# NUS-HPC-AI-Lab/VideoSys

Measured on AMD Instinct MI355X. Metric: videos/min (Open-Sora 512x512x64f, 30 denoise steps, DiT denoising only) + sec/denoise-step, higher is better.
Workload: dtype bf16; 1 GPU; open-sora-v1.2 STDiT3-XL/2 512x512x64f, latent [4,19,64,64], CFG batch 2 = 38912 token rows, 300 text tokens, depth 28; steps_per_video=30, parallelism=dsp1

## Files before the change

### videosys_amd/csrc/rowwise.hip

```cpp
#include "common.h"

#include <cstdlib>
#include "vsys_internal.h"

namespace vsys {
namespace {

template <int MAXV>
__global__ __launch_bounds__(256) void adaln_modulate_kernel(const bf16_t* __restrict__ x, const bf16_t* __restrict__ shift,
                                                             const bf16_t* __restrict__ scale, bf16_t* __restrict__ y,
                                                             int64_t rows, int C, int64_t rows_per_sample,
                                                             int64_t mod_stride, float eps) {
  const int lane = threadIdx.x & 63;
  const int64_t row = (int64_t)blockIdx.x * 4 + (threadIdx.x >> 6);
  if (row >= rows) return;
  const int nchunk = C >> 3;
  const bf16_t* xr = x + row * C;
  float v[MAXV][8];
  float s = 0.f;
#pragma unroll
  for (int i = 0; i < MAXV; ++i) {
    const int c = lane + 64 * i;
    if (c < nchunk) {
      uint4 u = *reinterpret_cast<const uint4*>(xr + c * 8);
      unpack8(u, v[i]);
#pragma unroll
      for (int e = 0; e < 8; ++e) s += v[i][e];
    }
  }
  const float mean = wave_sum(s) / (float)C;
  float q = 0.f;
#pragma unroll
  for (int i = 0; i < MAXV; ++i) {
    const int c = lane + 64 * i;
    if (c < nchunk) {
#pragma unroll
      for (int e = 0; e < 8; ++e) {
        float d = v[i][e] - mean;
        q += d * d;
      }
    }
  }
  const float rstd = rsqrtf(wave_sum(q) / (float)C + eps);
  const int64_t b = row / rows_per_sample;
  const bf16_t* sh = shift + b * mod_stride;
  const bf16_t* sc = scale + b * mod_stride;
  bf16_t* yr = y + row * C;
#pragma unroll
  for (int i = 0; i < MAXV; ++i) {
    const int c = lane + 64 * i;
    if (c < nchunk) {
      float a[8], m[8], o[8];
      unpack8(*reinterpret_cast<const uint4*>(sh + c * 8), a);
      unpack8(*reinterpret_cast<const uint4*>(sc + c * 8), m);
#pragma unroll
      for (int e = 0; e < 8; ++e) o[e] = (v[i][e] - mean) * rstd * (1.0f + m[e]) + a[e];
      *reinterpret_cast<uint4*>(yr + c * 8) = pack8(o);
    }
  }
}

template <int RPW>
__global__ __launch_bounds__(256) void adaln_modulate_rows_kernel(const bf16_t* __restrict__ x, const bf16_t* __restrict__ shift,
                                                                  const bf16_t* __restrict__ scale, bf16_t* __restrict__ y,
                                                                  int64_t rows, int C, int64_t rows_per_sample,
                                                                  int64_t mod_stride, float eps) {
  constexpr int MAXV = 3;
  const int lane = threadIdx.x & 63;
  const int64_t row0 = ((int64_t)blockIdx.x * 4 + (threadIdx.x >> 6)) * RPW;
  if (row0 >= rows) return;
  const int nchunk = C >> 3;
  uint4 u[RPW][MAXV];
#pragma unroll
  for (int r = 0; r < RPW; ++r) {
    const int64_t row = row0 + r < rows ? row0 + r : rows - 1;
#pragma unroll
    for (int i = 0; i < MAXV; ++i) {
      const int c = lane + 64 * i;
      u[r][i] = c < nchunk ? *reinterpret_cast<const uint4*>(x + row * C + c * 8) : make_uint4(0, 0, 0, 0);
    }
  }
  const int64_t b = row0 / rows_per_sample;
  uint4 ush[MAXV], usc[MAXV];
#pragma unroll
  for (int i = 0; i < MAXV; ++i) {
    const int c = lane + 64 * i;
    ush[i] = c < nchunk ? *reinterpret_cast<const uint4*>(shift + b * mod_stride + c * 8) : make_uint4(0, 0, 0, 0);
    usc[i] = c < nchunk ? *reinterpret_cast<const uint4*>(scale + b * mod_stride + c * 8) : make_uint4(0, 0, 0, 0);
  }
#pragma unroll
  for (int r = 0; r < RPW; ++r) {
    float v[MAXV][8];
    float s = 0.f;
#pragma unroll
    for (int i = 0; i < MAXV; ++i) {
      unpack8(u[r][i], v[i]);
      if (lane + 64 * i < nchunk) {
#pragma unroll
        for (int e = 0; e < 8; ++e) s += v[i][e];
      }
    }
    const float mean = wave_sum(s) / (float)C;
    float q = 0.f;
#pragma unroll
    for (int i = 0; i < MAXV; ++i) {
      if (lane + 64 * i < nchunk) {
#pragma unroll
        for (int e = 0; e < 8; ++e) {
          float d = v[i][e] - mean;
          q += d * d;
        }
      }
    }
    const float rstd = rsqrtf(wave_sum(q) / (float)C + eps);
    if (row0 + r < rows) {
#pragma unroll
      for (int i = 0; i < MAXV; ++i) {
        const int c = lane + 64 * i;
        if (c < nchunk) {
          float a[8], m[8], o[8];
          unpack8(ush[i], a);
          unpack8(usc[i], m);
#pragma unroll
          for (int e = 0; e < 8; ++e) o[e] = (v[i][e] - mean) * rstd * (1.0f + m[e]) + a[e];
          *reinterpret_cast<uint4*>(y + (row0 + r) * C + c * 8) = pack8(o);
        }
      }
    }
  }
}

template <int MAXV>
__global__ __launch_bounds__(256) void ln_modulate_kernel(const bf16_t* __restrict__ x, const bf16_t* __restrict__ ln_w,
                                                          const bf16_t* __restrict__ ln_b, const bf16_t* __restrict__ shift,
                                                          const bf16_t* __restrict__ scale, bf16_t* __restrict__ y, int64_t rows,
                                                          int C, int64_t rows_per_sample, int64_t mod_stride, int64_t seg_split,
                                                          int64_t mod_alt, float eps) {
  const int lane = threadIdx.x & 63;
  const int64_t row = (int64_t)blockIdx.x * 4 + (threadIdx.x >> 6);
  if (row >= rows) return;
  const int nchunk = C >> 3;
  const bf16_t* xr = x + row * C;
  float v[MAXV][8];
  float s = 0.f;
#pragma unroll
  for (int i = 0; i < MAXV; ++i) {
    const int c = lane + 64 * i;
    if (c < nchunk) {
      unpack8(*reinterpret_cast<const uint4*>(xr + c * 8), v[i]);
#pragma unroll
      for (int e = 0; e < 8; ++e) s += v[i][e];
    }
  }
  const float mean = wave_sum(s) / (float)C;
  float q = 0.f;
#pragma unroll
  for (int i = 0; i < MAXV; ++i) {
    const int c = lane + 64 * i;
    if (c < nchunk) {
#pragma unroll
      for (int e = 0; e < 8; ++e) {
        const float d = v[i][e] - mean;
        q += d * d;
      }
    }
  }
  const float rstd = rsqrtf(wave_sum(q) / (float)C + eps);
  const int64_t b = row / rows_per_sample;
  const int64_t alt = (seg_split > 0 && row - b * rows_per_sample < seg_split) ? mod_alt : 0;
  bf16_t* yr = y + row * C;
#pragma unroll
  for (int i = 0; i < MAXV; ++i) {
    const int c = lane + 64 * i;
    if (c < nchunk) {
      float o[8];
#pragma unroll
      for (int e = 0; e < 8; ++e) o[e] = (v[i][e] - mean) * rstd;
      if (ln_w != nullptr) {
        float w[8], bb[8];
        unpack8(*reinterpret_cast<const uint4*>(ln_w + c * 8), w);
        unpack8(*reinterpret_cast<const uint4*>(ln_b + c * 8), bb);
#pragma unroll
        for (int e = 0; e < 8; ++e) o[e] = o[e] * w[e] + bb[e];
      }
      if (shift != nullptr) {
        float a[8], m[8];
        unpack8(*reinterpret_cast<const uint4*>(shift + b * mod_stride + alt + c * 8), a);
        unpack8(*reinterpret_cast<const uint4*>(scale + b * mod_stride + alt + c * 8), m);
#pragma unroll
        for (int e = 0; e < 8; ++e) o[e] = o[e] * (1.0f + m[e]) + a[e];
      }
      *reinterpret_cast<uint4*>(yr + c * 8) = pack8(o);
    }
  }
}

__global__ void gate_add_rows_kernel(bf16_t* __restrict__ x, const bf16_t* __restrict__ y, const bf16_t* __restrict__ gate,
                                     int64_t rows, int C8, int64_t rows_per_sample, int64_t gate_stride, int64_t seg_split,
                                     int64_t gate_alt) {
  const int64_t total = rows * C8;
  for (int64_t i = (int64_t)blockIdx.x * blockDim.x + threadIdx.x; i < total; i += (int64_t)gridDim.x * blockDim.x) {
    const int64_t r = i / C8;
    const int c = (int)(i - r * C8);
    const int64_t b = r / rows_per_sample;
    const int64_t alt = (seg_split > 0 && r - b * rows_per_sample < seg_split) ? gate_alt : 0;
    float a[8], v[8], g[8];
    unpack8(reinterpret_cast<const uint4*>(x)[i], a);
    unpack8(reinterpret_cast<const uint4*>(y)[i], v);
    unpack8(*reinterpret_cast<const uint4*>(gate + b * gate_stride + alt + c * 8), g);
#pragma unroll
    for (int k = 0; k < 8; ++k) a[k] += bf2f(f2bf(g[k] * v[k]));
    reinterpret_cast<uint4*>(x)[i] = pack8(a);
  }
}

__global__ void im2col_patch_kernel(const float* __restrict__ z, int Bz, bf16_t* __restrict__ out, int B, int F, int Cin, int H,
                                    int W, int p) {
  const int Hp = H / p, Wp = W / p, K = Cin * p * p;
  const int64_t total = (int64_t)B * F * Hp * Wp * K;
  for (int64_t i = (int64_t)blockIdx.x * blockDim.x + threadIdx.x; i < total; i += (int64_t)gridDim.x * blockDim.x) {
    const int k = (int)(i % K);
    const int64_t tok = i / K;
    const int wp = (int)(tok % Wp), hp = (int)((tok / Wp) % Hp), f = (int)((tok / ((int64_t)Wp * Hp)) % F);
    const int b = (int)(tok / ((int64_t)Wp * Hp * F));
    const int dx = k % p, dy = (k / p) % p, c = k / (p * p);
    out[i] = f2bf(z[((((int64_t)(b % Bz) * F + f) * Cin + c) * H + hp * p + dy) * W + wp * p + dx]);
  }
}

__global__ void unpatchify_cvx_kernel(const bf16_t* __restrict__ x, int64_t ldx, float* __restrict__ out, int B, int F, int Hp,
                                      int Wp, int Cout, int p) {
  const int H = Hp * p, W = Wp * p;
  const int64_t total = (int64_t)B * F * Cout * H * W;
  for (int64_t i = (int64_t)blockIdx.x * blockDim.x + threadIdx.x; i < total; i += (int64_t)gridDim.x * blockDim.x) {
    const int w = (int)(i % W), h = (int)((i / W) % H), c = (int)((i / ((int64_t)W * H)) % Cout);
    const int64_t bf = i / ((int64_t)W * H * Cout);
    const int64_t tok = (bf * Hp + h / p) * Wp + w / p;
    out[i] = bf2f(x[tok * ldx + (c * p + h % p) * p + w % p]);
  }
}

__global__ void mod_table_kernel(const bf16_t* __restrict__ table, const bf16_t* __restrict__ t_mlp, bf16_t* __restrict__ out,
                                 int nblk, int B, int C6) {
  const int64_t i = (int64_t)blockIdx.x * blockDim.x + threadIdx.x;
  const int64_t total = (int64_t)nblk * B * C6;
  if (i >= total) return;
  const int c = (int)(i % C6);
  const int b = (int)((i / C6) % B);
  const int k = (int)(i / ((int64_t)C6 * B));
  out[i] = f2bf(bf2f(table[(int64_t)k * C6 + c]) + bf2f(t_mlp[(int64_t)b * C6 + c]));
}

__global__ void timestep_embedding_kernel(const float* __restrict__ t, bf16_t* __restrict__ out, int B, int dim) {
  const int i = blockIdx.x * blockDim.x + threadIdx.x;
  const int half = dim / 2;
  if (i >= B * half) return;
  const int b = i / half, k = i - b * half;
  const float f = expf(-9.210340371976184f * (float)k / (float)half);
  const float a = t[b] * f;
  out[(int64_t)b * dim + k] = f2bf(cosf(a));
  out[(int64_t)b * dim + half + k] = f2bf(sinf(a));
}

__global__ __launch_bounds__(256) void patch_embed_kernel(const float* __restrict__ x, int Bz, const bf16_t* __restrict__ w,
                                                          const bf16_t* __restrict__ bias, const bf16_t* __restrict__ pos,
                                                          bf16_t* __restrict__ out, int B, int Cin, int T, int H, int W,
                                                          int ph, int pw, int C, int s0, int Sl) {
  const int Hp = (H + ph - 1) / ph, Wp = (W + pw - 1) / pw;
  const int S = Hp * Wp;
  const int cchunks = C >> 3;
  const int64_t total = (int64_t)B * T * Sl * cchunks;
  const int64_t i = (int64_t)blockIdx.x * blockDim.x + threadIdx.x;
  if (i >= total) return;
  const int cc = (int)(i % cchunks);
  const int64_t tok = i / cchunks;
  const int s = s0 + (int)(tok % Sl);
  const int t = (int)((tok / Sl) % T);
  const int b = (int)(tok / ((int64_t)Sl * T));
  const int bz = b % Bz;
  if (s >= S) {
    *reinterpret_cast<uint4*>(out + tok * C + cc * 8) = make_uint4(0, 0, 0, 0);
    return;
  }
  const int hp = s / Wp, wp = s - hp * Wp;
  float acc[8];
  {
    float bb[8];
    unpack8(*reinterpret_cast<const uint4*>(bias + cc * 8), bb);
#pragma unroll
    for (int e = 0; e < 8; ++e) acc[e] = bb[e];
  }
  const int K = Cin * ph * pw;
  if (K == 16) {
    float xin[16];
#pragma unroll
    for (int k = 0; k < 16; ++k) {
      const int ci = k >> 2, dy = (k >> 1) & 1, dx = k & 1;
      const int hh = hp * 2 + dy, ww = wp * 2 + dx;
      xin[k] = 0.f;
      if (ph == 2 && pw == 2 && hh < H && ww < W) xin[k] = bf2f(f2bf(x[((((int64_t)bz * Cin + ci) * T + t) * H + hh) * W + ww]));
    }
    if (ph == 2 && pw == 2) {
#pragma unroll
      for (int e = 0; e < 8; ++e) {
        const bf16_t* wr = w + (int64_t)(cc * 8 + e) * 16;
        float wa[8], wb[8];
        unpack8(*reinterpret_cast<const uint4*>(wr), wa);
        unpack8(*reinterpret_cast<const uint4*>(wr + 8), wb);
#pragma unroll
        for (int k = 0; k < 8; ++k) acc[e] += xin[k] * wa[k] + xin[k + 8] * wb[k];
      }
    }
  }
  if (!(K == 16 && ph == 2 && pw == 2)) {
    for (int ci = 0; ci < Cin; ++ci)
      for (int dy = 0; dy < ph; ++dy)
        for (int dx = 0; dx < pw; ++dx) {
          const int hh = hp * ph + dy, ww = wp * pw + dx;
          float xv = 0.f;
          if (hh < H && ww < W) xv = bf2f(f2bf(x[((((int64_t)bz * Cin + ci) * T + t) * H + hh) * W + ww]));
          const int k = (ci * ph + dy) * pw + dx;
#pragma unroll
          for (int e = 0; e < 8; ++e) acc[e] += xv * bf2f(w[(int64_t)(cc * 8 + e) * K + k]);
        }
  }
  float pp[8];
  unpack8(*reinterpret_cast<const uint4*>(pos + (int64_t)s * C + cc * 8), pp);
#pragma unroll
  for (int e = 0; e < 8; ++e) acc[e] = bf2f(f2bf(acc[e])) + pp[e];
  *reinterpret_cast<uint4*>(out + tok * C + cc * 8) = pack8(acc);
}

template <int MAXV>
__global__ __launch_bounds__(256) void final_layer_kernel(const bf16_t* __restrict__ x, const bf16_t* __restrict__ table,
                                                          const bf16_t* __restrict__ tvec, const bf16_t* __restrict__ w,
                                                          const bf16_t* __restrict__ bias, float* __restrict__ out,
                                                          int B, int T, int Hp, int Wp, int H, int W, int ph, int pw,
                                                          int Cout, int C, float eps, int Sl, float* __restrict__ tokens) {
  const int lane = threadIdx.x & 63;
  const int S = Sl;
  const int64_t rows = (int64_t)B * T * S;
  const int64_t row = (int64_t)blockIdx.x * 4 + (threadIdx.x >> 6);
  if (row >= rows) return;
  const int nchunk = C >> 3;
  const bf16_t* xr = x + row * C;
  float v[MAXV][8];
  float s = 0.f;
#pragma unroll
  for (int i = 0; i < MAXV; ++i) {
    const int c = lane + 64 * i;
    if (c < nchunk) {
      unpack8(*reinterpret_cast<const uint4*>(xr + c * 8), v[i]);
#pragma unroll
      for (int e = 0; e < 8; ++e) s += v[i][e];
    } else {
#pragma unroll
      for (int e = 0; e < 8; ++e) v[i][e] = 0.f;
    }
  }
  const float mean = wave_sum(s) / (float)C;
  float q = 0.f;
#pragma unroll
  for (int i = 0; i < MAXV; ++i) {
    const int c = lane + 64 * i;
    if (c < nchunk) {
#pragma unroll
      for (int e = 0; e < 8; ++e) {
        float d = v[i][e] - mean;
        q += d * d;
      }
    }
  }
  const float rstd = rsqrtf(wave_sum(q) / (float)C + eps);
  const int b = (int)(row / ((int64_t)T * S));
#pragma unroll
  for (int i = 0; i < MAXV; ++i) {
    const int c = lane + 64 * i;
    if (c < nchunk) {
      float sh[8], sc[8], tt[8];
      unpack8(*reinterpret_cast<const uint4*>(table + c * 8), sh);
      unpack8(*reinterpret_cast<const uint4*>(table + C + c * 8), sc);
      unpack8(*reinterpret_cast<const uint4*>(tvec + (int64_t)b * C + c * 8), tt);
#pragma unroll
      for (int e = 0; e < 8; ++e) {
        const float shift = bf2f(f2bf(sh[e] + tt[e])), scale = bf2f(f2bf(sc[e] + tt[e]));
        v[i][e] = bf2f(f2bf((v[i][e] - mean) * rstd * (1.0f + scale) + shift));
      }
    }
  }
  const int NOUT = ph * pw * Cout;
  const int64_t tok = row % ((int64_t)T * S);
  const int t = (int)(tok / S), sidx = (int)(tok % S);
  const int hp = sidx / Wp, wp = sidx - hp * Wp;
  for (int n = 0; n < NOUT; ++n) {
    const bf16_t* wr = w + (int64_t)n * C;
    float d = 0.f;
#pragma unroll
    for (int i = 0; i < MAXV; ++i) {
      const int c = lane + 64 * i;
      if (c < nchunk) {
        float ww[8];
        unpack8(*reinterpret_cast<const uint4*>(wr + c * 8), ww);
#pragma unroll
        for (int e = 0; e < 8; ++e) d += v[i][e] * ww[e];
      }
    }
    d = wave_sum(d);
    if (lane == 0) {
      d = bf2f(f2bf(d + bf2f(bias[n])));
      if (tokens != nullptr) {
        tokens[row * NOUT + n] = d;
        continue;
      }
      const int co = n % Cout;
      const int dx = (n / Cout) % pw, dy = n / (Cout * pw);
      const int hh = hp * ph + dy, ww2 = wp * pw + dx;
      if (hh < H && ww2 < W) out[((((int64_t)b * Cout + co) * T + t) * H + hh) * W + ww2] = d;
    }
  }
}

__global__ void unpatchify_tokens_kernel(const float* __restrict__ tok, float* __restrict__ out, int P, int B, int T, int Sl,
                                         int Hp, int Wp, int H, int W, int ph, int pw, int Cout) {
  const int NOUT = ph * pw * Cout;
  const int64_t total = (int64_t)B * Cout * T * H * W;
  const int64_t i = (int64_t)blockIdx.x * blockDim.x + threadIdx.x;
  if (i >= total) return;
  const int ww = (int)(i % W), hh = (int)((i / W) % H), t = (int)((i / ((int64_t)W * H)) % T);
  const int co = (int)((i / ((int64_t)W * H * T)) % Cout), b = (int)(i / ((int64_t)W * H * T * Cout));
  const int hp = hh / ph, dy = hh - hp * ph, wp = ww / pw, dx = ww - wp * pw;
  const int s = hp * Wp + wp;
  const int r = s / Sl, j = s - r * Sl;
  const int n = (dy * pw + dx) * Cout + co;
  out[i] = tok[((((int64_t)r * B + b) * T + t) * Sl + j) * NOUT + n];
}

__global__ void cfg_euler_kernel(float* __restrict__ z, const float* __restrict__ model_out, int Bz, int Cin, int Cout,
                                 int64_t thw, float guidance, float dt) {
  const int64_t i = (int64_t)blockIdx.x * blockDim.x + threadIdx.x;
  const int64_t total = (int64_t)Bz * Cin * thw;
  if (i >= total) return;
  const int64_t sp = i % thw;
  const int c = (int)((i / thw) % Cin);
  const int b = (int)(i / (thw * Cin));
  const float cond = model_out[((int64_t)b * Cout + c) * thw + sp];
  const float unc = model_out[((int64_t)(b + Bz) * Cout + c) * thw + sp];
  z[i] = z[i] + (unc + guidance * (cond - unc)) * dt;
}

__global__ void cfg_axpby_kernel(float* __restrict__ z, const float* __restrict__ model_out, int Bz, int Cin, int Cout,
                                 int64_t thw, float guidance, float c_z, float c_eps, int cond_first) {
  const int64_t i = (int64_t)blockIdx.x * blockDim.x + threadIdx.x;
  const int64_t total = (int64_t)Bz * Cin * thw;
  if (i >= total) return;
  const int64_t sp = i % thw;
  const int c = (int)((i / thw) % Cin);
  const int b = (int)(i / (thw * Cin));
  const float h0 = model_out[((int64_t)b * Cout + c) * thw + sp];
  const float h1 = model_out[((int64_t)(b + Bz) * Cout + c) * thw + sp];
  const float cond = cond_first ? h0 : h1, unc = cond_first ? h1 : h0;
  z[i] = c_z * z[i] + c_eps * (unc + guidance * (cond - unc));
}

__global__ void add_bcast_rows_kernel(bf16_t* __restrict__ x, const bf16_t* __restrict__ e, int64_t rows, int C8, int64_t group,
                                      int64_t period) {
  const int64_t total = rows * C8;
  for (int64_t i = (int64_t)blockIdx.x * blockDim.x + threadIdx.x; i < total; i += (int64_t)gridDim.x * blockDim.x) {
    const int64_t r = i / C8;
    const int c = (int)(i - r * C8);
    const int64_t er = (r / group) % period;
    float a[8], b[8];
    unpack8(reinterpret_cast<const uint4*>(x)[i], a);
    unpack8(reinterpret_cast<const uint4*>(e)[er * C8 + c], b);
#pragma unroll
    for (int k = 0; k < 8; ++k) a[k] += b[k];
    reinterpret_cast<uint4*>(x)[i] = pack8(a);
  }
}

__global__ void add_rows_kernel(bf16_t* __restrict__ x, const bf16_t* __restrict__ y, int64_t n8) {
  for (int64_t i = (int64_t)blockIdx.x * blockDim.x + threadIdx.x; i < n8; i += (int64_t)gridDim.x * blockDim.x) {
    float a[8], b[8];
    unpack8(reinterpret_cast<const uint4*>(x)[i], a);
    unpack8(reinterpret_cast<const uint4*>(y)[i], b);
#pragma unroll
    for (int e = 0; e < 8; ++e) a[e] += b[e];
    reinterpret_cast<uint4*>(x)[i] = pack8(a);
  }
}

__global__ void scale_add_rows_kernel(const bf16_t* __restrict__ a, int64_t lda, const bf16_t* __restrict__ b, int64_t ldb,
                                      bf16_t* __restrict__ out, int64_t ldo, int64_t rows, int C8, float scale) {
  const int64_t total = rows * C8;
  for (int64_t i = (int64_t)blockIdx.x * blockDim.x + threadIdx.x; i < total; i += (int64_t)gridDim.x * blockDim.x) {
    const int64_t r = i / C8;
    const int c = (int)(i - r * C8) * 8;
    float x[8], y[8];
    unpack8(*reinterpret_cast<const uint4*>(a + r * lda + c), x);
    unpack8(*reinterpret_cast<const uint4*>(b + r * ldb + c), y);
#pragma unroll
    for (int e = 0; e < 8; ++e) x[e] = bf2f(f2bf(x[e] * scale)) + y[e];
    *reinterpret_cast<uint4*>(out + r * ldo + c) = pack8(x);
  }
}

__global__ void copy_4d_kernel(const bf16_t* __restrict__ src, bf16_t* __restrict__ dst, int n0, int n1, int n2, int C,
                               int64_t ss0, int64_t ss1, int64_t ss2, int64_t ds0, int64_t ds1, int64_t ds2,
                               int n1_valid, int n2_valid) {
  const int cch = C >> 3;
  const int64_t total = (int64_t)n0 * n1 * n2 * cch;
  for (int64_t i = (int64_t)blockIdx.x * blockDim.x + threadIdx.x; i < total; i += (int64_t)gridDim.x * blockDim.x) {
    const int c = (int)(i % cch);
    int64_t r = i / cch;
    const int i2 = (int)(r % n2);
    r /= n2;
    const int i1 = (int)(r % n1);
    const int i0 = (int)(r / n1);
    uint4 v = make_uint4(0, 0, 0, 0);
    if (i1 < n1_valid && i2 < n2_valid) v = *reinterpret_cast<const uint4*>(src + i0 * ss0 + i1 * ss1 + i2 * ss2 + c * 8);
    *reinterpret_cast<uint4*>(dst + i0 * ds0 + i1 * ds1 + i2 * ds2 + c * 8) = v;
  }
}

struct CopyBatch {
  int nops;
  CopyDesc d[VSYS_COPY_BATCH_MAX];
};
__global__ void copy_4d_batch_kernel(const bf16_t* __restrict__ src, bf16_t* __restrict__ dst, CopyBatch b) {
  const CopyDesc& o = b.d[blockIdx.y];
  const int cch = o.C >> 3;
  const int64_t total = (int64_t)o.n0 * o.n1 * o.n2 * cch;
  const bf16_t* s = src + o.src_off;
  bf16_t* d = dst + o.dst_off;
  for (int64_t i = (int64_t)blockIdx.x * blockDim.x + threadIdx.x; i < total; i += (int64_t)gridDim.x * blockDim.x) {
    const int c = (int)(i % cch);
    int64_t r = i / cch;
    const int i2 = (int)(r % o.n2);
    r /= o.n2;
    const int i1 = (int)(r % o.n1);
    const int i0 = (int)(r / o.n1);
    uint4 v = make_uint4(0, 0, 0, 0);
    if (i1 < o.n1_valid && i2 < o.n2_valid) v = *reinterpret_cast<const uint4*>(s + i0 * o.ss0 + i1 * o.ss1 + i2 * o.ss2 + c * 8);
    *reinterpret_cast<uint4*>(d + i0 * o.ds0 + i1 * o.ds1 + i2 * o.ds2 + c * 8) = v;
  }
}

}

int launch_copy_4d_batch(const bf16_t* src, bf16_t* dst, const CopyDesc* ops, int nops, hipStream_t stream) {
  if (nops <= 0) return 0;
  if (nops > VSYS_COPY_BATCH_MAX) return VSYS_ERR_SHAPE;
  CopyBatch b;
  b.nops = nops;
  int64_t most = 0;
  for (int i = 0; i < nops; ++i) {
    if (ops[i].C % 8 || ops[i].n0 < 0 || ops[i].n1 < 0 || ops[i].n2 < 0) return VSYS_ERR_SHAPE;
    b.d[i] = ops[i];
    const int64_t t = (int64_t)ops[i].n0 * ops[i].n1 * ops[i].n2 * (ops[i].C / 8);
    most = t > most ? t : most;
  }
  if (most <= 0) return 0;
  int64_t grid = (most + 255) / 256;
  if (grid > 2048) grid = 2048;
  hipLaunchKernelGGL(copy_4d_batch_kernel, dim3((unsigned)grid, (unsigned)nops), dim3(256), 0, stream, src, dst, b);
  return hipGetLastError() == hipSuccess ? 0 : VSYS_ERR_LAUNCH;
}

int launch_adaln_modulate(const bf16_t* x, const bf16_t* shift, const bf16_t* scale, bf16_t* y, int64_t rows, int C,
                          int64_t rows_per_sample, int64_t mod_stride, float eps, hipStream_t stream) {
  if (rows <= 0) return 0;
  if (C % 8 != 0 || C > 64 * 8 * 4 || rows_per_sample <= 0 || (mod_stride % 8)) return VSYS_ERR_SHAPE;
  if (C > 64 * 8 * 2 && C <= 64 * 8 * 3 && rows_per_sample % 2 == 0) {
    hipLaunchKernelGGL(adaln_modulate_rows_kernel<2>, dim3((unsigned)((rows + 7) / 8)), dim3(256), 0, stream, x, shift, scale, y, rows, C,
                       rows_per_sample, mod_stride, eps);
    return hipGetLastError() == hipSuccess ? 0 : VSYS_ERR_LAUNCH;
  }
  const unsigned grid = (unsigned)((rows + 3) / 4);
  if (C <= 64 * 8 * 2)
    hipLaunchKernelGGL(adaln_modulate_kernel<2>, dim3(grid), dim3(256), 0, stream, x, shift, scale, y, rows, C,
                       rows_per_sample, mod_stride, eps);
  else if (C <= 64 * 8 * 3)
    hipLaunchKernelGGL(adaln_modulate_kernel<3>, dim3(grid), dim3(256), 0, stream, x, shift, scale, y, rows, C,
                       rows_per_sample, mod_stride, eps);
  else
    hipLaunchKernelGGL(adaln_modulate_kernel<4>, dim3(grid), dim3(256), 0, stream, x, shift, scale, y, rows, C,
                       rows_per_sample, mod_stride, eps);
  return hipGetLastError() == hipSuccess ? 0 : VSYS_ERR_LAUNCH;
}

int launch_ln_modulate(const bf16_t* x, const bf16_t* ln_w, const bf16_t* ln_b, const bf16_t* shift, const bf16_t* scale,
                       bf16_t* y, int64_t rows, int C, int64_t rows_per_sample, int64_t mod_stride, int64_t seg_split,
                       int64_t mod_alt, float eps, hipStream_t stream) {
  if (rows <= 0) return 0;
  if (C % 8 != 0 || C > 64 * 8 * 6 || rows_per_sample <= 0 || (mod_stride % 8) || (mod_alt % 8)) return VSYS_ERR_SHAPE;
  if ((ln_w == nullptr) != (ln_b == nullptr) || (shift == nullptr) != (scale == nullptr)) return VSYS_ERR_ARG;
  const unsigned grid = (unsigned)((rows + 3) / 4);
#define VSYS_LNMOD(V)                                                                                                      \
  hipLaunchKernelGGL(ln_modulate_kernel<V>, dim3(grid), dim3(256), 0, stream, x, ln_w, ln_b, shift, scale, y, rows, C,       \
                     rows_per_sample, mod_stride, seg_split, mod_alt, eps)
  if (C <= 64 * 8 * 2) VSYS_LNMOD(2);
  else if (C <= 64 * 8 * 3) VSYS_LNMOD(3);
  else if (C <= 64 * 8 * 4) VSYS_LNMOD(4);
  else VSYS_LNMOD(6);
#undef VSYS_LNMOD
  return hipGetLastError() == hipSuccess ? 0 : VSYS_ERR_LAUNCH;
}

int launch_gate_add_rows(bf16_t* x, const bf16_t* y, const bf16_t* gate, int64_t rows, int C, int64_t rows_per_sample,
                         int64_t gate_stride, int64_t seg_split, int64_t gate_alt, hipStream_t stream) {
  if (rows <= 0) return 0;
  if (C % 8 || rows_per_sample <= 0 || (gate_stride % 8) || (gate_alt % 8)) return VSYS_ERR_SHAPE;
  int64_t grid = (rows * (C / 8) + 255) / 256;
  if (grid > 2048 * 4) grid = 2048 * 4;
  hipLaunchKernelGGL(gate_add_rows_kernel, dim3((unsigned)grid), dim3(256), 0, stream, x, y, gate, rows, C / 8, rows_per_sample,
                     gate_stride, seg_split, gate_alt);
  return hipGetLastError() == hipSuccess ? 0 : VSYS_ERR_LAUNCH;
}

int launch_im2col_patch(const float* z, int Bz, bf16_t* out, int B, int F, int Cin, int H, int W, int p, hipStream_t stream) {
  if (p <= 0 || H % p || W % p || Bz <= 0) return VSYS_ERR_SHAPE;
  const int64_t total = (int64_t)B * F * (H / p) * (W / p) * Cin * p * p;
  if (total <= 0) return 0;
  int64_t grid = (total + 255) / 256;
  if (grid > 2048 * 8) grid = 2048 * 8;
  hipLaunchKernelGGL(im2col_patch_kernel, dim3((unsigned)grid), dim3(256), 0, stream, z, Bz, out, B, F, Cin, H, W, p);
  return hipGetLastError() == hipSuccess ? 0 : VSYS_ERR_LAUNCH;
}

int launch_unpatchify_cvx(const bf16_t* x, int64_t ldx, float* out, int B, int F, int Hp, int Wp, int Cout, int p,
                          hipStream_t stream) {
  const int64_t total = (int64_t)B * F * Cout * Hp * p * Wp * p;
  if (total <= 0) return 0;
  int64_t grid = (total + 255) / 256;
  if (grid > 2048 * 8) grid = 2048 * 8;
  hipLaunchKernelGGL(unpatchify_cvx_kernel, dim3((unsigned)grid), dim3(256), 0, stream, x, ldx, out, B, F, Hp, Wp, Cout, p);
  return hipGetLastError() == hipSuccess ? 0 : VSYS_ERR_LAUNCH;
}

int launch_mod_table(const bf16_t* table, const bf16_t* t_mlp, bf16_t* out, int nblk, int B, int C6, hipStream_t stream) {
  const int64_t total = (int64_t)nblk * B * C6;
  if (total <= 0) return 0;
  hipLaunchKernelGGL(mod_table_kernel, dim3((unsigned)((total + 255) / 256)), dim3(256), 0, stream, table, t_mlp, out, nblk,
                     B, C6);
  return hipGetLastError() == hipSuccess ? 0 : VSYS_ERR_LAUNCH;
}

int launch_timestep_embedding(const float* t, bf16_t* out, int B, int dim, hipStream_t stream) {
  if (dim % 2) return VSYS_ERR_SHAPE;
  const int total = B * (dim / 2);
  if (total <= 0) return 0;
  hipLaunchKernelGGL(timestep_embedding_kernel, dim3((total + 127) / 128), dim3(128), 0, stream, t, out, B, dim);
  return hipGetLastError() == hipSuccess ? 0 : VSYS_ERR_LAUNCH;
}

int launch_patch_embed(const float* x, int Bz, const bf16_t* w, const bf16_t* bias, const bf16_t* pos, bf16_t* out, int B,
                       int Cin, int T, int H, int W, int ph, int pw, int C, int s0, int Sl, hipStream_t stream) {
  if (C % 8 || Bz <= 0 || s0 < 0) return VSYS_ERR_SHAPE;
  const int Hp = (H + ph - 1) / ph, Wp = (W + pw - 1) / pw;
  if (Sl < 0) Sl = Hp * Wp;
  const int64_t total = (int64_t)B * T * Sl * (C / 8);
  if (total <= 0) return 0;
  if ((total + 255) / 256 > 0x7fffffff) return VSYS_ERR_SHAPE;
  hipLaunchKernelGGL(patch_embed_kernel, dim3((unsigned)((total + 255) / 256)), dim3(256), 0, stream, x, Bz, w, bias, pos, out,
                     B, Cin, T, H, W, ph, pw, C, s0, Sl);
  return hipGetLastError() == hipSuccess ? 0 : VSYS_ERR_LAUNCH;
}

int launch_unpatchify_tokens(const float* tok, float* out, int P, int B, int T, int Sl, int Hp, int Wp, int H, int W, int ph,
                             int pw, int Cout, hipStream_t stream) {
  if (P <= 0 || Sl <= 0 || (int64_t)P * Sl < (int64_t)Hp * Wp) return VSYS_ERR_SHAPE;
  const int64_t total = (int64_t)B * Cout * T * H * W;
  if (total <= 0) return 0;
  if ((total + 255) / 256 > 0x7fffffff) return VSYS_ERR_SHAPE;
  hipLaunchKernelGGL(unpatchify_tokens_kernel, dim3((unsigned)((total + 255) / 256)), dim3(256), 0, stream, tok, out, P, B, T, Sl,
                     Hp, Wp, H, W, ph, pw, Cout);
  return hipGetLastError() == hipSuccess ? 0 : VSYS_ERR_LAUNCH;
}

int launch_final_layer(const bf16_t* x, const bf16_t* table, const bf16_t* tvec, const bf16_t* w, const bf16_t* bias,
                       float* out, int B, int T, int Hp, int Wp, int H, int W, int ph, int pw, int Cout, int C, float eps,
                       int Sl, float* tokens, hipStream_t stream) {
  if (C % 8 != 0 || C > 64 * 8 * 4) return VSYS_ERR_SHAPE;
  if (Sl < 0) Sl = Hp * Wp;
  if (tokens == nullptr && Sl != Hp * Wp) return VSYS_ERR_ARG;
  const int64_t rows = (int64_t)B * T * Sl;
  if (rows <= 0) return 0;
  const unsigned grid = (unsigned)((rows + 3) / 4);
  if (C <= 64 * 8 * 2)
    hipLaunchKernelGGL(final_layer_kernel<2>, dim3(grid), dim3(256), 0, stream, x, table, tvec, w, bias, out, B, T, Hp, Wp,
                       H, W, ph, pw, Cout, C, eps, Sl, tokens);
  else if (C <= 64 * 8 * 3)
    hipLaunchKernelGGL(final_layer_kernel<3>, dim3(grid), dim3(256), 0, stream, x, table, tvec, w, bias, out, B, T, Hp, Wp,
                       H, W, ph, pw, Cout, C, eps, Sl, tokens);
  else
    hipLaunchKernelGGL(final_layer_kernel<4>, dim3(grid), dim3(256), 0, stream, x, table, tvec, w, bias, out, B, T, Hp, Wp,
                       H, W, ph, pw, Cout, C, eps, Sl, tokens);
  return hipGetLastError() == hipSuccess ? 0 : VSYS_ERR_LAUNCH;
}

int launch_cfg_euler(float* z, const float* model_out, int Bz, int Cin, int Cout, int64_t thw, float guidance, float dt,
                     hipStream_t stream) {
  const int64_t total = (int64_t)Bz * Cin * thw;
  if (total <= 0) return 0;
  hipLaunchKernelGGL(cfg_euler_kernel, dim3((unsigned)((total + 255) / 256)), dim3(256), 0, stream, z, model_out, Bz, Cin,
                     Cout, thw, guidance, dt);
  return hipGetLastError() == hipSuccess ? 0 : VSYS_ERR_LAUNCH;
}

int launch_cfg_axpby(float* z, const float* model_out, int Bz, int Cin, int Cout, int64_t thw, float guidance, float c_z,
                     float c_eps, int cond_first, hipStream_t stream) {
  const int64_t total = (int64_t)Bz * Cin * thw;
  if (total <= 0) return 0;
  hipLaunchKernelGGL(cfg_axpby_kernel, dim3((unsigned)((total + 255) / 256)), dim3(256), 0, stream, z, model_out, Bz, Cin,
                     Cout, thw, guidance, c_z, c_eps, cond_first);
  return hipGetLastError() == hipSuccess ? 0 : VSYS_ERR_LAUNCH;
}

int launch_add_bcast_rows(bf16_t* x, const bf16_t* e, int64_t rows, int C, int64_t group, int64_t period, hipStream_t stream) {
  if (rows <= 0) return 0;
  if (C % 8 || group <= 0 || period <= 0) return VSYS_ERR_SHAPE;
  int64_t grid = (rows * (C / 8) + 255) / 256;
  if (grid > 2048 * 4) grid = 2048 * 4;
  hipLaunchKernelGGL(add_bcast_rows_kernel, dim3((unsigned)grid), dim3(256), 0, stream, x, e, rows, C / 8, group, period);
  return hipGetLastError() == hipSuccess ? 0 : VSYS_ERR_LAUNCH;
}

int launch_add_rows(bf16_t* x, const bf16_t* y, int64_t n, hipStream_t stream) {
  if (n <= 0) return 0;
  if (n % 8) return VSYS_ERR_SHAPE;
  const int64_t n8 = n / 8;
  int64_t grid = (n8 + 255) / 256;
  if (grid > 2048 * 4) grid = 2048 * 4;
  hipLaunchKernelGGL(add_rows_kernel, dim3((unsigned)grid), dim3(256), 0, stream, x, y, n8);
  return hipGetLastError() == hipSuccess ? 0 : VSYS_ERR_LAUNCH;
}

int launch_scale_add_rows(const bf16_t* a, int64_t lda, const bf16_t* b, int64_t ldb, bf16_t* out, int64_t ldo, int64_t rows, int C,
                          float scale, hipStream_t stream) {
  if (rows < 0 || C < 0) return VSYS_ERR_SHAPE;
  if (rows == 0 || C == 0) return 0;
  if (C % 8 || lda < C || ldb < C || ldo < C) return VSYS_ERR_SHAPE;
  if ((lda % 8) || (ldb % 8) || (ldo % 8) || reinterpret_cast<uintptr_t>(a) % 16 || reinterpret_cast<uintptr_t>(b) % 16 ||
      reinterpret_cast<uintptr_t>(out) % 16)
    return VSYS_ERR_ALIGN;
  int64_t grid = (rows * (C / 8) + 255) / 256;
  if (grid > 2048 * 4) grid = 2048 * 4;
  hipLaunchKernelGGL(scale_add_rows_kernel, dim3((unsigned)grid), dim3(256), 0, stream, a, lda, b, ldb, out, ldo, rows, C / 8, scale);
  return hipGetLastError() == hipSuccess ? 0 : VSYS_ERR_LAUNCH;
}

int launch_copy_4d(const bf16_t* src, bf16_t* dst, int n0, int n1, int n2, int C, int64_t ss0, int64_t ss1, int64_t ss2,
                   int64_t ds0, int64_t ds1, int64_t ds2, int n1_valid, int n2_valid, hipStream_t stream) {
  if (C % 8) return VSYS_ERR_SHAPE;
  const int64_t total = (int64_t)n0 * n1 * n2 * (C / 8);
  if (total <= 0) return 0;
  int64_t grid = (total + 255) / 256;
  if (grid > 2048 * 4) grid = 2048 * 4;
  hipLaunchKernelGGL(copy_4d_kernel, dim3((unsigned)grid), dim3(256), 0, stream, src, dst, n0, n1, n2, C, ss0, ss1, ss2, ds0,
                     ds1, ds2, n1_valid, n2_valid);
  return hipGetLastError() == hipSuccess ? 0 : VSYS_ERR_LAUNCH;
}

}
```

Measured before the change: 21.42 videos/min.

## Add specialized patch-embed and final-layer kernels with register/LDS weight reuse

Adds a persistent patch-embed kernel for the 2x2, 4-channel case. It keeps the 16-wide weight rows in registers, double-buffers the input patches through shared memory and processes several tokens per block. It also adds a persistent final-layer kernel that stages the projection weights in LDS, handles four rows per wave and reduces across output channels with a shuffle tree. Both aim to cut redundant weight loads and per-row reductions in two kernels that run once per denoise step. They are small next to the 28 transformer blocks, so they add code complexity and hand-written asm in exchange for a small end-to-end gain.

```diff
diff --git a/videosys_amd/csrc/rowwise.hip b/videosys_amd/csrc/rowwise.hip
--- a/videosys_amd/csrc/rowwise.hip
+++ b/videosys_amd/csrc/rowwise.hip
@@ -262,7 +262,7 @@
   out[(int64_t)b * dim + half + k] = f2bf(sinf(a));
 }
 
-__global__ __launch_bounds__(256) void patch_embed_kernel(const float* __restrict__ x, int Bz, const bf16_t* __restrict__ w,
+__global__ __launch_bounds__(256) void patch_embed_ref_kernel(const float* __restrict__ x, int Bz, const bf16_t* __restrict__ w,
                                                           const bf16_t* __restrict__ bias, const bf16_t* __restrict__ pos,
                                                           bf16_t* __restrict__ out, int B, int Cin, int T, int H, int W,
                                                           int ph, int pw, int C, int s0, int Sl) {
@@ -331,8 +331,181 @@
   *reinterpret_cast<uint4*>(out + tok * C + cc * 8) = pack8(acc);
 }
 
+
+__device__ __forceinline__ void pe_quad(float (&acc)[8], int e0, const float (&xm)[4], const float (&wm)[4], const float (&xf)[4],
+                                        const float (&wf)[4]) {
+  float t0, t1, t2, t3;
+  asm("v_mul_f32_e32 %[t0], %[xm0], %[wm0]\n\t"
+      "v_mul_f32_e32 %[t1], %[xm1], %[wm1]\n\t"
+      "v_mul_f32_e32 %[t2], %[xm2], %[wm2]\n\t"
+      "v_mul_f32_e32 %[t3], %[xm3], %[wm3]\n\t"
+      "v_fmac_f32_e32 %[t0], %[xf0], %[wf0]\n\t"
+      "v_fmac_f32_e32 %[t1], %[xf1], %[wf1]\n\t"
+      "v_fmac_f32_e32 %[t2], %[xf2], %[wf2]\n\t"
+      "v_fmac_f32_e32 %[t3], %[xf3], %[wf3]\n\t"
+      "v_add_f32_e32 %[a0], %[t0], %[a0]\n\t"
+      "v_add_f32_e32 %[a1], %[t1], %[a1]\n\t"
+      "v_add_f32_e32 %[a2], %[t2], %[a2]\n\t"
+      "v_add_f32_e32 %[a3], %[t3], %[a3]"
+      : [a0] "+v"(acc[e0]), [a1] "+v"(acc[e0 + 1]), [a2] "+v"(acc[e0 + 2]), [a3] "+v"(acc[e0 + 3]), [t0] "=&v"(t0), [t1] "=&v"(t1),
+        [t2] "=&v"(t2), [t3] "=&v"(t3)
+      : [xm0] "v"(xm[0]), [xm1] "v"(xm[1]), [xm2] "v"(xm[2]), [xm3] "v"(xm[3]), [wm0] "v"(wm[0]), [wm1] "v"(wm[1]), [wm2] "v"(wm[2]),
+        [wm3] "v"(wm[3]), [xf0] "v"(xf[0]), [xf1] "v"(xf[1]), [xf2] "v"(xf[2]), [xf3] "v"(xf[3]), [wf0] "v"(wf[0]), [wf1] "v"(wf[1]),
+        [wf2] "v"(wf[2]), [wf3] "v"(wf[3]));
+}
+__device__ __forceinline__ void fl_mac2x4(float (&res)[4], float a00, float a01, float a02, float a03, float w0, float a10, float a11,
+                                          float a12, float a13, float w1) {
+  float t0, t1, t2, t3;
+  asm("v_mul_f32_e32 %[t0], %[a00], %[w0]\n\t"
+      "v_mul_f32_e32 %[t1], %[a01], %[w0]\n\t"
+      "v_mul_f32_e32 %[t2], %[a02], %[w0]\n\t"
+      "v_mul_f32_e32 %[t3], %[a03], %[w0]\n\t"
+      "v_add_f32_e32 %[r0], %[r0], %[t0]\n\t"
+      "v_add_f32_e32 %[r1], %[r1], %[t1]\n\t"
+      "v_add_f32_e32 %[r2], %[r2], %[t2]\n\t"
+      "v_add_f32_e32 %[r3], %[r3], %[t3]\n\t"
+      "v_mul_f32_e32 %[t0], %[a10], %[w1]\n\t"
+      "v_mul_f32_e32 %[t1], %[a11], %[w1]\n\t"
+      "v_mul_f32_e32 %[t2], %[a12], %[w1]\n\t"
+      "v_mul_f32_e32 %[t3], %[a13], %[w1]\n\t"
+      "v_add_f32_e32 %[r0], %[r0], %[t0]\n\t"
+      "v_add_f32_e32 %[r1], %[r1], %[t1]\n\t"
+      "v_add_f32_e32 %[r2], %[r2], %[t2]\n\t"
+      "v_add_f32_e32 %[r3], %[r3], %[t3]"
+      : [r0] "+v"(res[0]), [r1] "+v"(res[1]), [r2] "+v"(res[2]), [r3] "+v"(res[3]), [t0] "=&v"(t0), [t1] "=&v"(t1), [t2] "=&v"(t2),
+        [t3] "=&v"(t3)
+      : [a00] "v"(a00), [a01] "v"(a01), [a02] "v"(a02), [a03] "v"(a03), [w0] "v"(w0), [a10] "v"(a10), [a11] "v"(a11), [a12] "v"(a12),
+        [a13] "v"(a13), [w1] "v"(w1));
+}
+
+constexpr int PE_TJ = 4;
+constexpr int PE_MAXSLOTS = 8;
+constexpr int PE_LPT = 4;
+
+constexpr int PE_NONE = -1, PE_PAD = -2;
+__device__ __forceinline__ float pe_input(const float* __restrict__ x, int Bz, int T, int H, int W, int Wp, int S, int s0, int Sl,
+                                          int ntok, int tok, int k, int& state, bool& ok) {
+  const bool there = tok < ntok;
+  const unsigned ut = there ? (unsigned)tok : 0u;
+  const unsigned bt = ut / (unsigned)Sl;
+  const int s = s0 + (int)(ut - bt * (unsigned)Sl);
+  state = there ? (s < S ? s : PE_PAD) : PE_NONE;
+  const int sc = s < S ? s : 0;
+  const unsigned b = bt / (unsigned)T;
+  const int t = (int)(bt - b * (unsigned)T);
+  const int bz = (int)(b % (unsigned)Bz);
+  const int hp = (int)((unsigned)sc / (unsigned)Wp), wp = sc - hp * Wp;
+  const int ci = k >> 2, dy = (k >> 1) & 1, dx = k & 1;
+  const int hh = hp * 2 + dy, ww = wp * 2 + dx;
+  ok = there && s < S && hh < H && ww < W;
+  const int64_t idx = ok ? ((((int64_t)bz * 4 + ci) * T + t) * H + hh) * W + ww : 0;
+  return x[idx];
+}
+
+__global__ __launch_bounds__(512) void patch_embed_k16_kernel(const float* __restrict__ x, int Bz, const bf16_t* __restrict__ w,
+                                                              const bf16_t* __restrict__ bias, const bf16_t* __restrict__ pos,
+                                                              bf16_t* __restrict__ out, int B, int T, int H, int W, int C, int s0,
+                                                              int Sl, int nslots) {
+#pragma clang fp contract(off)
+  __shared__ __attribute__((aligned(16))) float xs[2][PE_TJ * PE_MAXSLOTS][16];
+  __shared__ int ss[2][PE_TJ * PE_MAXSLOTS];
+  const int Hp = (H + 1) / 2, Wp = (W + 1) / 2;
+  const int S = Hp * Wp;
+  const int cchunks = C >> 3;
+  const int ntok = B * T * Sl;
+  const int tid = threadIdx.x;
+  const int slot = tid / cchunks;
+  const bool active = slot < nslots;
+  const int cc = active ? tid - slot * cchunks : 0;
+  const int tpi = nslots * PE_TJ, nload = tpi * 16;
+
+  float wa[8][8], wb[8][8], bb[8];
+#pragma unroll
+  for (int e = 0; e < 8; ++e) {
+    const bf16_t* wr = w + (int64_t)(cc * 8 + e) * 16;
+    unpack8(*reinterpret_cast<const uint4*>(wr), wa[e]);
+    unpack8(*reinterpret_cast<const uint4*>(wr + 8), wb[e]);
+  }
+  unpack8(*reinterpret_cast<const uint4*>(bias + cc * 8), bb);
+
+  int tok0 = (int)blockIdx.x * tpi;
+  const int step = (int)gridDim.x * tpi;
+  float xv[PE_LPT];
+  int sv[PE_LPT];
+  bool okv[PE_LPT];
+#pragma unroll
+  for (int q = 0; q < PE_LPT; ++q) {
+    const int l = tid + q * (int)blockDim.x;
+    xv[q] = 0.f;
+    sv[q] = PE_NONE;
+    okv[q] = false;
+    if (l < nload) {
+      xv[q] = pe_input(x, Bz, T, H, W, Wp, S, s0, Sl, ntok, tok0 + (l >> 4), l & 15, sv[q], okv[q]);
+      xs[0][l >> 4][l & 15] = okv[q] ? bf2f(f2bf(xv[q])) : 0.f;
+      if ((l & 15) == 0) ss[0][l >> 4] = sv[q];
+    }
+  }
+  __syncthreads();
+  int buf = 0;
+  for (; tok0 < ntok; tok0 += step, buf ^= 1) {
+#pragma unroll
+    for (int q = 0; q < PE_LPT; ++q) {
+      const int l = tid + q * (int)blockDim.x;
+      if (l < nload) xv[q] = pe_input(x, Bz, T, H, W, Wp, S, s0, Sl, ntok, tok0 + step + (l >> 4), l & 15, sv[q], okv[q]);
+    }
+    int st[PE_TJ];
+    uint4 up[PE_TJ];
+    if (active) {
+#pragma unroll
+      for (int j = 0; j < PE_TJ; ++j) {
+        st[j] = ss[buf][j * nslots + slot];
+        up[j] = make_uint4(0, 0, 0, 0);
+        if (st[j] >= 0) up[j] = *reinterpret_cast<const uint4*>(pos + (int64_t)st[j] * C + cc * 8);
+      }
+#pragma unroll
+      for (int j = 0; j < PE_TJ; ++j) {
+        const int tl = j * nslots + slot;
+        float xin[16];
+#pragma unroll
+        for (int v4 = 0; v4 < 4; ++v4) {
+          const float4 f = reinterpret_cast<const float4*>(xs[buf][tl])[v4];
+          xin[4 * v4] = f.x; xin[4 * v4 + 1] = f.y; xin[4 * v4 + 2] = f.z; xin[4 * v4 + 3] = f.w;
+        }
+        float acc[8];
+#pragma unroll
+        for (int e = 0; e < 8; ++e) acc[e] = bb[e];
+#pragma unroll
+        for (int k = 0; k < 8; ++k) {
+          const float lo = xin[k], hi = xin[k + 8];
+          pe_quad(acc, 0, {lo, hi, lo, hi}, {wa[0][k], wb[1][k], wa[2][k], wb[3][k]}, {hi, lo, hi, lo}, {wb[0][k], wa[1][k], wb[2][k], wa[3][k]});
+          pe_quad(acc, 4, {lo, hi, hi, hi}, {wa[4][k], wb[5][k], wb[6][k], wb[7][k]}, {hi, lo, lo, lo}, {wb[4][k], wa[5][k], wa[6][k], wa[7][k]});
+        }
+        float pp[8], o[8];
+        unpack8(up[j], pp);
+#pragma unroll
+        for (int e = 0; e < 8; ++e) o[e] = bf2f(f2bf(acc[e])) + pp[e];
+        up[j] = st[j] == PE_PAD ? make_uint4(0, 0, 0, 0) : pack8(o);
+      }
+    }
+#pragma unroll
+    for (int q = 0; q < PE_LPT; ++q) {
+      const int l = tid + q * (int)blockDim.x;
+      if (l < nload) {
+        xs[buf ^ 1][l >> 4][l & 15] = okv[q] ? bf2f(f2bf(xv[q])) : 0.f;
+        if ((l & 15) == 0) ss[buf ^ 1][l >> 4] = sv[q];
+      }
+    }
+    if (active) {
+#pragma unroll
+      for (int j = 0; j < PE_TJ; ++j)
+        if (st[j] != PE_NONE) *reinterpret_cast<uint4*>(out + (int64_t)(tok0 + j * nslots + slot) * C + cc * 8) = up[j];
+    }
+    __syncthreads();
+  }
+}
+
 template <int MAXV>
-__global__ __launch_bounds__(256) void final_layer_kernel(const bf16_t* __restrict__ x, const bf16_t* __restrict__ table,
+__global__ __launch_bounds__(256) void final_layer_ref_kernel(const bf16_t* __restrict__ x, const bf16_t* __restrict__ table,
                                                           const bf16_t* __restrict__ tvec, const bf16_t* __restrict__ w,
                                                           const bf16_t* __restrict__ bias, float* __restrict__ out,
                                                           int B, int T, int Hp, int Wp, int H, int W, int ph, int pw,
@@ -416,6 +589,192 @@
       const int dx = (n / Cout) % pw, dy = n / (Cout * pw);
       const int hh = hp * ph + dy, ww2 = wp * pw + dx;
       if (hh < H && ww2 < W) out[((((int64_t)b * Cout + co) * T + t) * H + hh) * W + ww2] = d;
+    }
+  }
+}
+
+constexpr int FL_R = 4;
+
+template <int LVL, int MAXV>
+__device__ __forceinline__ void fl_tree(const float (&a)[FL_R][MAXV][8], const uint4* lw, int n, int NOUT, int nchunk, int lane,
+                                        const int (&lbase)[MAXV], const int (&lmul)[MAXV], float (&res)[FL_R]) {
+#pragma clang fp contract(off)
+  if constexpr (LVL == 0) {
+#pragma unroll
+    for (int r = 0; r < FL_R; ++r) res[r] = 0.f;
+    const int rowoff = (n < NOUT ? n : NOUT) * nchunk;
+#pragma unroll
+    for (int i = 0; i < MAXV; ++i) {
+      float ww[8];
+      unpack8(lw[lbase[i] + lmul[i] * rowoff], ww);
+#pragma unroll
+      for (int e = 0; e < 8; e += 2)
+        fl_mac2x4(res, a[0][i][e], a[1][i][e], a[2][i][e], a[3][i][e], ww[e], a[0][i][e + 1], a[1][i][e + 1], a[2][i][e + 1], a[3][i][e + 1],
+                  ww[e + 1]);
+    }
+  } else {
+    float lo[FL_R], hi[FL_R];
+    fl_tree<LVL - 1, MAXV>(a, lw, n, NOUT, nchunk, lane, lbase, lmul, lo);
+    fl_tree<LVL - 1, MAXV>(a, lw, n + (1 << (LVL - 1)), NOUT, nchunk, lane, lbase, lmul, hi);
+    constexpr int o = 64 >> LVL;
+    const bool up = (lane & o) != 0;
+#pragma unroll
+    for (int r = 0; r < FL_R; ++r) {
+      const float keep = up ? hi[r] : lo[r], send = up ? lo[r] : hi[r];
+      res[r] = keep + __shfl_xor(send, o, 64);
+    }
+  }
+}
+
+__device__ __forceinline__ void fl_wave_sums(float (&v)[FL_R]) {
+#pragma clang fp contract(off)
+#pragma unroll
+  for (int o = 32; o > 0; o >>= 1) {
+    float t[FL_R];
+#pragma unroll
+    for (int r = 0; r < FL_R; ++r) t[r] = __shfl_xor(v[r], o, 64);
+#pragma unroll
+    for (int r = 0; r < FL_R; ++r) v[r] = v[r] + t[r];
+  }
+}
+
+template <int MAXV>
+__global__ __launch_bounds__(256) void final_layer_kernel(const bf16_t* __restrict__ x, const bf16_t* __restrict__ table,
+                                                          const bf16_t* __restrict__ tvec, const bf16_t* __restrict__ w,
+                                                          const bf16_t* __restrict__ bias, float* __restrict__ out,
+                                                          int B, int T, int Hp, int Wp, int H, int W, int ph, int pw,
+                                                          int Cout, int C, float eps, int Sl, float* __restrict__ tokens) {
+#pragma clang fp contract(off)
+  extern __shared__ __attribute__((aligned(16))) uint4 fl_w[];
+  const int lane = threadIdx.x & 63;
+  const int wave = __builtin_amdgcn_readfirstlane((int)(threadIdx.x >> 6));
+  const int nchunk = C >> 3;
+  const int NOUT = ph * pw * Cout;
+  const int S = Sl;
+  const int64_t rows = (int64_t)B * T * S;
+  for (int i = threadIdx.x; i < (NOUT + 1) * nchunk; i += 256)
+    fl_w[i] = i < NOUT * nchunk ? reinterpret_cast<const uint4*>(w)[i] : make_uint4(0, 0, 0, 0);
+  __syncthreads();
+  int lbase[MAXV], lmul[MAXV];
+#pragma unroll
+  for (int i = 0; i < MAXV; ++i) {
+    const int c = lane + 64 * i;
+    lmul[i] = c < nchunk ? 1 : 0;
+    lbase[i] = c < nchunk ? c : NOUT * nchunk;
+  }
+  const int nl = ((lane >> 5) & 1) | (((lane >> 4) & 1) << 1) | (((lane >> 3) & 1) << 2) | (((lane >> 2) & 1) << 3) | (((lane >> 1) & 1) << 4);
+  const int64_t ngroups = (rows + FL_R - 1) / FL_R;
+  const float fC = (float)C;
+  for (int64_t g = (int64_t)blockIdx.x * 4 + wave; g < ngroups; g += (int64_t)gridDim.x * 4) {
+    const int64_t row0 = g * FL_R;
+    uint4 u[FL_R][MAXV];
+    int bs[FL_R];
+#pragma unroll
+    for (int r = 0; r < FL_R; ++r) {
+      const int64_t row = row0 + r < rows ? row0 + r : rows - 1;
+      bs[r] = (int)(row / ((int64_t)T * S));
+#pragma unroll
+      for (int i = 0; i < MAXV; ++i) {
+        const int c = lane + 64 * i;
+        u[r][i] = c < nchunk ? *reinterpret_cast<const uint4*>(x + row * C + c * 8) : make_uint4(0, 0, 0, 0);
+      }
+    }
+    float a[FL_R][MAXV][8];
+    float st[FL_R];
+#pragma unroll
+    for (int r = 0; r < FL_R; ++r) {
+      st[r] = 0.f;
+#pragma unroll
+      for (int i = 0; i < MAXV; ++i) {
+        unpack8(u[r][i], a[r][i]);
+        if (lane + 64 * i < nchunk) {
+#pragma unroll
+          for (int e = 0; e < 8; ++e) st[r] = st[r] + a[r][i][e];
+        }
+      }
+    }
+    fl_wave_sums(st);
+    float mean[FL_R];
+#pragma unroll
+    for (int r = 0; r < FL_R; ++r) {
+      mean[r] = st[r] / fC;
+      st[r] = 0.f;
+#pragma unroll
+      for (int i = 0; i < MAXV; ++i) {
+        if (lane + 64 * i < nchunk) {
+#pragma unroll
+          for (int e = 0; e < 8; ++e) {
+            const float d = a[r][i][e] - mean[r];
+            const float dd = d * d;
+            st[r] = st[r] + dd;
+          }
+        }
+      }
+    }
+    fl_wave_sums(st);
+    float rstd[FL_R];
+#pragma unroll
+    for (int r = 0; r < FL_R; ++r) rstd[r] = rsqrtf(st[r] / fC + eps);
+    const int b0 = bs[0];
+#pragma unroll
+    for (int i = 0; i < MAXV; ++i) {
+      const int c = lane + 64 * i;
+      if (c < nchunk) {
+        float sh[8], sc[8], t0[8];
+        unpack8(*reinterpret_cast<const uint4*>(table + c * 8), sh);
+        unpack8(*reinterpret_cast<const uint4*>(table + C + c * 8), sc);
+        unpack8(*reinterpret_cast<const uint4*>(tvec + (int64_t)b0 * C + c * 8), t0);
+        float shift0[8], scale0[8];
+#pragma unroll
+        for (int e = 0; e < 8; ++e) {
+          shift0[e] = bf2f(f2bf(sh[e] + t0[e]));
+          scale0[e] = 1.0f + bf2f(f2bf(sc[e] + t0[e]));
+        }
+#pragma unroll
+        for (int r = 0; r < FL_R; ++r) {
+          if (bs[r] == b0) {
+#pragma unroll
+            for (int e = 0; e < 8; ++e) {
+              const float t = (a[r][i][e] - mean[r]) * rstd[r];
+              a[r][i][e] = bf2f(f2bf(__builtin_fmaf(t, scale0[e], shift0[e])));
+            }
+          } else {
+            float t1[8];
+            unpack8(*reinterpret_cast<const uint4*>(tvec + (int64_t)bs[r] * C + c * 8), t1);
+#pragma unroll
+            for (int e = 0; e < 8; ++e) {
+              const float shift = bf2f(f2bf(sh[e] + t1[e])), scale = bf2f(f2bf(sc[e] + t1[e]));
+              const float t = (a[r][i][e] - mean[r]) * rstd[r];
+              a[r][i][e] = bf2f(f2bf(__builtin_fmaf(t, 1.0f + scale, shift)));
+            }
+          }
+        }
+      }
+    }
+    for (int n0 = 0; n0 < NOUT; n0 += 32) {
+      float res[FL_R];
+      fl_tree<5, MAXV>(a, fl_w, n0, NOUT, nchunk, lane, lbase, lmul, res);
+      const int n = n0 + nl;
+      const float bn = n < NOUT ? bf2f(bias[n]) : 0.f;
+#pragma unroll
+      for (int r = 0; r < FL_R; ++r) {
+        float d = res[r] + __shfl_xor(res[r], 1, 64);
+        const int64_t row = row0 + r;
+        if ((lane & 1) || n >= NOUT || row >= rows) continue;
+        d = bf2f(f2bf(d + bn));
+        if (tokens != nullptr) {
+          tokens[row * NOUT + n] = d;
+          continue;
+        }
+        const int b = bs[r];
+        const int64_t tok = row - (int64_t)b * T * S;
+        const int t = (int)(tok / S), sidx = (int)(tok - (int64_t)t * S);
+        const int hp = sidx / Wp, wp = sidx - hp * Wp;
+        const int co = n % Cout;
+        const int dx = (n / Cout) % pw, dy = n / (Cout * pw);
+        const int hh = hp * ph + dy, ww2 = wp * pw + dx;
+        if (hh < H && ww2 < W) out[((((int64_t)b * Cout + co) * T + t) * H + hh) * W + ww2] = d;
+      }
     }
   }
 }
@@ -547,6 +906,11 @@
 
 }
 
+static bool rowwise_ref() {
+  static const bool on = [] { const char* e = getenv("VSYS_ROWWISE_REF"); return e && e[0] == '1'; }();
+  return on;
+}
+
 int launch_copy_4d_batch(const bf16_t* src, bf16_t* dst, const CopyDesc* ops, int nops, hipStream_t stream) {
   if (nops <= 0) return 0;
   if (nops > VSYS_COPY_BATCH_MAX) return VSYS_ERR_SHAPE;
@@ -661,7 +1025,22 @@
   const int64_t total = (int64_t)B * T * Sl * (C / 8);
   if (total <= 0) return 0;
   if ((total + 255) / 256 > 0x7fffffff) return VSYS_ERR_SHAPE;
-  hipLaunchKernelGGL(patch_embed_kernel, dim3((unsigned)((total + 255) / 256)), dim3(256), 0, stream, x, Bz, w, bias, pos, out,
+  const int cchunks = C / 8;
+  if (!rowwise_ref() && Cin == 4 && ph == 2 && pw == 2 && cchunks * PE_LPT >= PE_TJ * 16 && cchunks <= 512 &&
+      (int64_t)B * T * Sl < (1 << 30)) {
+    int nslots = 1, threads = (cchunks + 63) / 64 * 64;
+    for (int ns = 2; ns <= PE_MAXSLOTS && ns * cchunks <= 512; ++ns) {
+      const int th = (ns * cchunks + 63) / 64 * 64;
+      if ((int64_t)ns * cchunks * threads >= (int64_t)nslots * cchunks * th) nslots = ns, threads = th;
+    }
+    const int64_t ntok = (int64_t)B * T * Sl, tpi = (int64_t)nslots * PE_TJ;
+    int64_t grid = (ntok + tpi - 1) / tpi;
+    if (grid > cu_count_this_device()) grid = cu_count_this_device();
+    hipLaunchKernelGGL(patch_embed_k16_kernel, dim3((unsigned)grid), dim3((unsigned)threads), 0, stream, x, Bz, w, bias, pos, out, B, T, H,
+                       W, C, s0, Sl, nslots);
+    return hipGetLastError() == hipSuccess ? 0 : VSYS_ERR_LAUNCH;
+  }
+  hipLaunchKernelGGL(patch_embed_ref_kernel, dim3((unsigned)((total + 255) / 256)), dim3(256), 0, stream, x, Bz, w, bias, pos, out,
                      B, Cin, T, H, W, ph, pw, C, s0, Sl);
   return hipGetLastError() == hipSuccess ? 0 : VSYS_ERR_LAUNCH;
 }
@@ -685,15 +1064,35 @@
   if (tokens == nullptr && Sl != Hp * Wp) return VSYS_ERR_ARG;
   const int64_t rows = (int64_t)B * T * Sl;
   if (rows <= 0) return 0;
+  const int64_t lds = ((int64_t)ph * pw * Cout + 1) * C * 2;
+  if (!rowwise_ref() && lds > 0 && lds <= 80 * 1024) {
+    static const bool attr = [] {
+      (void)hipFuncSetAttribute((const void*)final_layer_kernel<2>, hipFuncAttributeMaxDynamicSharedMemorySize, 80 * 1024);
+      (void)hipFuncSetAttribute((const void*)final_layer_kernel<3>, hipFuncAttributeMaxDynamicSharedMemorySize, 80 * 1024);
+      (void)hipFuncSetAttribute((const void*)final_layer_kernel<4>, hipFuncAttributeMaxDynamicSharedMemorySize, 80 * 1024);
+      return true;
+    }();
+    (void)attr;
+    int64_t pg = ((rows + FL_R - 1) / FL_R + 3) / 4;
+    if (pg > 2 * cu_count_this_device()) pg = 2 * cu_count_this_device();
+#define VSYS_FINAL(V)                                                                                                          \
+  hipLaunchKernelGGL(final_layer_kernel<V>, dim3((unsigned)pg), dim3(256), (size_t)lds, stream, x, table, tvec, w, bias, out, B, T, Hp, \
+                     Wp, H, W, ph, pw, Cout, C, eps, Sl, tokens)
+    if (C <= 64 * 8 * 2) VSYS_FINAL(2);
+    else if (C <= 64 * 8 * 3) VSYS_FINAL(3);
+    else VSYS_FINAL(4);
+#undef VSYS_FINAL
+    return hipGetLastError() == hipSuccess ? 0 : VSYS_ERR_LAUNCH;
+  }
   const unsigned grid = (unsigned)((rows + 3) / 4);
   if (C <= 64 * 8 * 2)
-    hipLaunchKernelGGL(final_layer_kernel<2>, dim3(grid), dim3(256), 0, stream, x, table, tvec, w, bias, out, B, T, Hp, Wp,
+    hipLaunchKernelGGL(final_layer_ref_kernel<2>, dim3(grid), dim3(256), 0, stream, x, table, tvec, w, bias, out, B, T, Hp, Wp,
                        H, W, ph, pw, Cout, C, eps, Sl, tokens);
   else if (C <= 64 * 8 * 3)
-    hipLaunchKernelGGL(final_layer_kernel<3>, dim3(grid), dim3(256), 0, stream, x, table, tvec, w, bias, out, B, T, Hp, Wp,
+    hipLaunchKernelGGL(final_layer_ref_kernel<3>, dim3(grid), dim3(256), 0, stream, x, table, tvec, w, bias, out, B, T, Hp, Wp,
                        H, W, ph, pw, Cout, C, eps, Sl, tokens);
   else
-    hipLaunchKernelGGL(final_layer_kernel<4>, dim3(grid), dim3(256), 0, stream, x, table, tvec, w, bias, out, B, T, Hp, Wp,
+    hipLaunchKernelGGL(final_layer_ref_kernel<4>, dim3(grid), dim3(256), 0, stream, x, table, tvec, w, bias, out, B, T, Hp, Wp,
                        H, W, ph, pw, Cout, C, eps, Sl, tokens);
   return hipGetLastError() == hipSuccess ? 0 : VSYS_ERR_LAUNCH;
 }
```

After: 21.56 videos/min, median of 6. About the same (+0.7%).
